# Luckick/EAGCN

Hardware: AMD Instinct MI355X
Metric: molecules/sec fwd+bwd, 2-layer 5-view EAGCN, Tox21 batch (higher is better)
Workload: dtype f32 (bf16x3 split, fp32 accumulate): every fp32 operand leaves its producer as three bf16 planes, six v_mfma_f32_32x32x16_bf16 piece products per 16 k rebuild the fp32 product (csrc/gemm_bx3.hip); aggregation, BatchNorm, head, first layer fp32

## Files before the change

eagcn_amd/_lib.py:

```python
import ctypes as C
import os

_HERE = os.path.dirname(os.path.abspath(__file__))
LIB_PATH = os.path.join(_HERE, 'lib', 'libeagcn_hip.so')

MAX_VIEWS = 8
MAX_SEGS = 8
META_WORDS = 16
META_NLOG = 8
META_T, META_NMAX, META_NTILES, META_BAD_ADJ, META_BAD_REL, META_NEDGE, META_OVERFLOW, META_EDGE_OVERFLOW = range(8)
META_NBLK = 9
STRUCT_CONCATE, STRUCT_WEIGHTED = 0, 1

_fp = C.c_void_p


class Batch(C.Structure):
    _fields_ = [('B', C.c_int32), ('N', C.c_int32), ('K', C.c_int32), ('ldc', C.c_int32),
                ('T', C.c_int32), ('n_max', C.c_int32), ('n_tiles', C.c_int32),
                ('channels', C.c_int32 * MAX_VIEWS),
                ('code', _fp), ('deg_bn', _fp), ('nat', _fp), ('row0', _fp), ('tile0', _fp),
                ('meta', _fp), ('row_mol', _fp), ('row_loc', _fp), ('row_m', _fp), ('row_deg', _fp),
                ('tile_mol', _fp), ('row_info', _fp), ('tile_info', _fp),
                ('rel_vec', _fp * MAX_VIEWS), ('rel_c', C.c_int32 * MAX_VIEWS),
# ... 176 lines not shown
    'eagcn_stream_signal_flag': (C.c_int, [_fp, _fp]),
    'eagcn_stream_wait_flag': (C.c_int, [_fp, C.c_double, _fp]),
    'eagcn_stream_wait_timeouts': (C.c_int, []),
    'eagcn_stream_wait_reset': (None, []),
    'eagcn_adam_step': (C.c_int, [_fp, _fp, _fp, _fp, C.c_int64, _fp, _fp, _fp, _fp]),
    'eagcn_grad_norm_workspace_bytes': (C.c_size_t, []),
    'eagcn_grad_norm': (C.c_int, [_fp, _fp, C.c_int64, _fp, C.c_int, _fp]),
    'eagcn_adam_step_clipped': (C.c_int, [_fp, _fp, _fp, _fp, C.c_int64, _fp, _fp, _fp, _fp, _fp, _fp, _fp]),
    'eagcn_agg_wants_bond_lists': (C.c_int, [C.c_int, C.c_int]),
    'eagcn_agg_wants_bond_lists_for': (C.c_int, [C.c_int, C.c_int, C.c_int]),
    'eagcn_bx3_used_splits': (C.c_int, [C.c_int, C.c_int, C.c_int, C.c_int]),
    'eagcn_set_bx3_wide': (C.c_int, [C.c_int]),
    'eagcn_set_top_bn_sums': (C.c_int, [C.c_int]),
    'eagcn_set_hidden_bn_sums': (C.c_int, [C.c_int]),
    'eagcn_hidden_bn_sums_taken': (C.c_long, [C.c_int]),
    'eagcn_bx3_pair_used_splits': (C.c_int, [C.c_int] * 7),
    'eagcn_bx3_plane_elems': (C.c_size_t, [C.c_int, C.c_int]),
    'eagcn_bx3_split': (C.c_int, [_fp, C.c_int, C.c_int, _fp, C.c_size_t, C.c_int, C.c_int, _fp]),
    'eagcn_gemm_bx3': (C.c_int, [C.c_int, C.c_int, C.c_int, C.c_int, _fp, C.c_size_t, C.c_int, C.c_int, _fp, C.c_size_t, C.c_int, C.c_int,
                                 _fp, C.c_int, C.c_int, C.c_size_t, C.c_int, _fp]),
    'eagcn_gemm_bx3_pair': (C.c_int, [C.c_int, C.c_int, C.c_int, _fp, C.c_size_t, C.c_int, C.c_int, _fp, C.c_size_t, C.c_int, C.c_int, _fp, C.c_int,
                                      C.c_int, C.c_int, C.c_int, _fp, C.c_size_t, C.c_int, C.c_int, _fp, C.c_size_t, C.c_int, C.c_int, _fp, C.c_int,
                                      C.c_int, C.c_size_t, C.c_int, _fp]),
    'eagcn_pack_rows': (C.c_int, [C.POINTER(Batch), _fp, C.c_int, C.POINTER(Layout), _fp, _fp]),
    'eagcn_unpack_rows': (C.c_int, [C.POINTER(Batch), _fp, C.POINTER(Layout), _fp, _fp, C.c_int, _fp]),
    'eagcn_pad_rows': (C.c_int, [_fp, _fp, C.c_int, C.c_int, C.c_int, _fp, _fp]),
    'eagcn_gat_scratch_bytes': (C.c_size_t, [C.POINTER(Batch), C.c_int]),
    'eagcn_gat_forward': (C.c_int, [C.POINTER(Batch), C.POINTER(GatParams), _fp, _fp, _fp, _fp, _fp]),
    'eagcn_gat_backward': (C.c_int, [C.POINTER(Batch), C.POINTER(GatParams), _fp, _fp, _fp, _fp, _fp, _fp, _fp, _fp, _fp,
                                     C.c_size_t, _fp]),
# ... 145 lines not shown
```

eagcn_amd/build.py:

```python
import os
import shutil
import subprocess
import sys
from concurrent.futures import ThreadPoolExecutor

HERE = os.path.dirname(os.path.abspath(__file__))
CSRC = os.path.join(HERE, 'csrc')
LIBDIR = os.path.join(HERE, 'lib')
LIB = os.path.join(LIBDIR, 'libeagcn_hip.so')
HIP_SOURCES = ['index.hip', 'gemm.hip', 'gemm3.hip', 'gemm_bx3.hip', 'gemm_bx3w.hip', 'agg.hip', 'lagg.hip', 'lagg_in.hip', 'lagg_top.hip', 'gat.hip', 'pool.hip', 'layer.hip', 'readout.hip', 'head.hip', 'head2.hip', 'loss.hip', 'clip.hip', 'attr.hip', 'metrics.hip', 'reps.hip']
CPP_SOURCES = ['api.cpp']
HEADERS = ['common.h', 'kernels.h', 'lagg_kernel.h', 'gemm_x6.h', 'bx3.h', 'bx3_epi.h', os.path.join('..', '..', 'include', 'eagcn_hip.h')]
ARCH = 'gfx950'


def _hipcc():
    for cand in (shutil.which('hipcc'), '/opt/rocm/bin/hipcc'):
        if cand and os.path.exists(cand):
            return cand
    raise RuntimeError('hipcc not found: the EAGCN HIP library cannot be built')


def _newest(paths):
    return max(os.path.getmtime(p) for p in paths)

# ... 46 lines not shown
```

eagcn_amd/csrc/kernels.h:

```cpp
#pragma once
#include "bx3.h"
#include "common.h"

namespace eagcn {

struct AggArgs {
    eagcn_batch bt;
    ViewCols vc;
    const float* src; int lds;
    float* dst; int ldd;
    const float* sig;
    const float* rsig;
    float* rscale;
    double* stats;
    int nchunk;
    int cpw = 1;
    int xcd = 0;
    bool w_rowm = false;
    bool w_gather = false;
    BxOut planes = {nullptr, 0, 0, 0};
    const float* bn_tab = nullptr; const float* bn_cc = nullptr; int bn_fp = 0;
    const float* w_aw = nullptr;
    int w_drop = 0; uint32_t w_thr = 0; float w_inv_keep = 1.0f; uint64_t w_seed = 0; const uint64_t* w_seed_dev = nullptr;
};
struct DropArgs { int on; uint32_t thr; float inv_keep; uint64_t seed; const uint64_t* seed_dev; };
inline DropArgs drop_args(float p, bool training, uint64_t seed, const uint64_t* seed_dev) {
    const double thr = (double)p * 4294967296.0;
    return DropArgs{(training && p > 0.0f) ? 1 : 0, (uint32_t)(thr < 4294967295.0 ? thr : 4294967295.0), 1.0f / (1.0f - p), seed, seed_dev};
}
inline void agg_set_drop(AggArgs& a, const DropArgs& d) {
    a.w_drop = d.on; a.w_thr = d.thr; a.w_inv_keep = d.inv_keep; a.w_seed = d.seed; a.w_seed_dev = d.seed_dev;
}
int agg_grid_x(const eagcn_batch* b);
bool agg_ksplit(const eagcn_batch* b);
int launch_agg(AggArgs a, bool trans, hipStream_t s);
constexpr int LAGG_RB = 256;
constexpr int LAGG_MAXM = 16;
struct EdgeArgs;
int lagg_parts();
bool lagg_wfuse();
bool lagg_use(const eagcn_batch* b, int dir, bool absorbs_bn, const ViewCols* vc = nullptr);
bool lagg_wanted(int B, int N, int structure);
int lagg_block_rows(const eagcn_batch* b);
int lagg_slabs(const eagcn_batch* b);
int launch_lagg_fwd(AggArgs a, hipStream_t s);
int launch_lagg_bwd(AggArgs a, const EdgeArgs& e, hipStream_t s, bool edge = true);
int launch_lagg_bwd_input(const AggArgs& a, const EdgeArgs& e, dim3 grid, hipStream_t s);
int launch_lagg_bwd_top(const AggArgs& a, const EdgeArgs& e, dim3 grid, hipStream_t s);

struct EdgeArgs {
    eagcn_batch bt;
    ViewCols vc;
    const float* dY; const float* Y; const float* P; int ld;
    const float* sig; const float* rsig; const float* rscale;
    double* datt;
    int atomic;
    int xcd = 0;
};
constexpr int EDGE_SLAB = 264;
constexpr int EDGE_COPIES = 8;
inline size_t edge_acc_bytes() { return align256((size_t)EDGE_COPIES * EAGCN_MAX_VIEWS * EDGE_SLAB * sizeof(double)); }
int edge_grid_x(const eagcn_batch* b);
int launch_agg_edge(AggArgs a, const EdgeArgs& e, hipStream_t s);
// ... 213 lines not shown
```

eagcn_amd/csrc/lagg.hip:

```cpp
#include <stdlib.h>

#include <algorithm>

#include "common.h"
#include "kernels.h"
#include "lagg_kernel.h"

namespace eagcn {


static int lagg_cpw(const eagcn_batch& bt, const ViewCols& vc, bool trans);
static int lagg_policy() {
    static const int v = [] {
        const char* e = getenv("EAGCN_AGG");
        if (e && !strcmp(e, "lds")) return 1;
        if (e && !strcmp(e, "dense")) return 0;
        return 2;
    }();
    return v;
}
static int lagg_min_n() {
    static const int v = env_int("EAGCN_LAGG_MIN_N", 240);
    return v;
}
// ... 46 lines not shown
    int chunks, gy;
    lagg_extent(bt, vc, &chunks, &gy);
    const long wgs = (long)vc.K * chunks * gy;
    int per = (trans && !cpw_bwd) ? 1 : cpw_env > 0 ? cpw_env : (int)std::min<long>(trans ? 4 : 8, std::max<long>(1, wgs / 3072));
    return std::max(1, std::min(per, chunks));
}
static int lagg_grid(const AggArgs& a, dim3* grid, int* nchunk, int* cpw, bool trans) {
    int chunks, gy;
    lagg_extent(a.bt, a.vc, &chunks, &gy);
    *cpw = lagg_cpw(a.bt, a.vc, trans);
    *nchunk = cdiv(chunks, *cpw);
    *grid = dim3((unsigned)(a.vc.K * *nchunk), (unsigned)gy);
    return EAGCN_OK;
}

int launch_lagg_fwd(AggArgs a, hipStream_t s) {
    if (a.bt.B == 0 || a.bt.T == 0) return EAGCN_OK;
    dim3 grid;
    int rc = lagg_grid(a, &grid, &a.nchunk, &a.cpw, false);
    if (rc) return rc;
    ProfScope ps(PROF_AGG, s);
    EdgeArgs e;
    memset(&e, 0, sizeof(e));
    if (a.cpw > 1) lagg_kernel<false, true><<<grid, 256, 0, s>>>(a, e);
    else lagg_kernel<false, false><<<grid, 256, 0, s>>>(a, e);
    EAGCN_LAUNCH_CHECK();
    return EAGCN_OK;
}

int launch_lagg_bwd(AggArgs a, const EdgeArgs& e, hipStream_t s, bool edge) {
    if (a.bt.B == 0 || a.bt.T == 0) return EAGCN_OK;
    EAGCN_CHECK_ARG(!edge || (e.atomic && e.datt), "lagg: the edge gradients leave through the shared accumulator slabs (EdgeArgs.atomic)");
    dim3 grid;
    int rc = lagg_grid(a, &grid, &a.nchunk, &a.cpw, true);
    if (rc) return rc;
    ProfScope ps(PROF_AGG, s);
    EAGCN_CHECK_ARG(!a.w_aw || a.bn_tab, "lagg: the upstream-gradient form needs the BatchNorm tables");
    EAGCN_CHECK_ARG(!a.w_rowm || a.bn_tab, "lagg: the row-mask staging needs the BatchNorm tables");
    if (!edge) {
        rc = launch_lagg_bwd_input(a, e, grid, s);
        if (rc) return rc;
    } else if (a.w_rowm) {
        rc = launch_lagg_bwd_top(a, e, grid, s);
        if (rc) return rc;
    } else if (a.w_aw) {
        lagg_kernel<true, true, true><<<grid, 256, 0, s>>>(a, e);
    } else {
        if (a.cpw > 1) lagg_kernel<true, true><<<grid, 256, 0, s>>>(a, e);
        else lagg_kernel<true, false><<<grid, 256, 0, s>>>(a, e);
    }
    EAGCN_LAUNCH_CHECK();
    return EAGCN_OK;
}

}

extern "C" int eagcn_agg_wants_bond_lists(int B, int N) { return eagcn::lagg_wanted(B, N, -1) ? 1 : 0; }
extern "C" int eagcn_agg_wants_bond_lists_for(int B, int N, int structure) { return eagcn::lagg_wanted(B, N, structure) ? 1 : 0; }
```

eagcn_amd/csrc/lagg_kernel.h:

```cpp
#pragma once

#include "common.h"
#include "kernels.h"

namespace eagcn {

constexpr int LG_CW = 32;
constexpr int LG_LPR = LG_CW / 4;
constexpr int LG_G = 256 / LG_LPR;
constexpr int LG_U = LAGG_RB / LG_G;
constexpr int LG_ECAP = 768;
constexpr int LG_EPT = LG_ECAP / 256;
constexpr bool LG_MERGE = true;
constexpr int LG_PJ_EARLY = 4;

__device__ __forceinline__ void lg_fma(float4& acc, float w, const float4& v) {
    acc.x = fmaf(w, v.x, acc.x); acc.y = fmaf(w, v.y, acc.y); acc.z = fmaf(w, v.z, acc.z); acc.w = fmaf(w, v.w, acc.w);
}
__device__ __forceinline__ void lg_add(float4& acc, const float4& v) { acc.x += v.x; acc.y += v.y; acc.z += v.z; acc.w += v.w; }
__device__ __forceinline__ float lg_dot(const float4& a, const float4& b) { return fmaf(a.x, b.x, fmaf(a.y, b.y, fmaf(a.z, b.z, a.w * b.w))); }
template <int CTRL>
__device__ __forceinline__ float lg_dpp(float v) {
    return __int_as_float(__builtin_amdgcn_update_dpp(0, __float_as_int(v), CTRL, 0xF, 0xF, true));
}
__device__ __forceinline__ float lg_gsum(float v) {
    v += lg_dpp<0xB1>(v); v += lg_dpp<0x4E>(v); v += lg_dpp<0x141>(v);
    return v;
}

struct LgLists {
    unsigned short nb[LG_ECAP];
    float w[LG_ECAP];
    unsigned char cd[LG_ECAP];
};
constexpr uint32_t LG_SLOW = 1u << 28;
constexpr uint32_t LG_OVF = 1u << 29;
constexpr int LG_NOVF = 32;

template <bool TRANS, bool MULTI, bool WFUSE = false, bool EDGE = true, bool CROWS = false, bool GATHER = false>
__global__ __launch_bounds__(256) __attribute__((amdgpu_waves_per_eu(3, 8))) void lagg_kernel(AggArgs a, EdgeArgs ed) {
    static_assert(TRANS || !WFUSE, "the upstream-gradient form belongs to the transposed kernel");
    static_assert(TRANS || EDGE, "the forward has no edge gradients to drop");
    static_assert(!CROWS || WFUSE, "the row-mask staging is a form of the upstream-gradient staging");
    static_assert(!GATHER || (CROWS && EDGE && MULTI), "the per-molecule gather is a form of the row-mask staging with the edge gradients");
    constexpr bool TE = TRANS && EDGE;
    constexpr int NREC = TRANS ? 3 : 2;
    __shared__ float4 buf[LAGG_RB][LG_LPR];
    __shared__ float4 s_rec[LAGG_RB][NREC];
    __shared__ float4 s_ovf[LG_NOVF][NREC];
    __shared__ int s_novf;
    __shared__ __attribute__((aligned(16))) unsigned char s_lists_raw[TRANS ? 16 : sizeof(LgLists)];
    __shared__ float s_rs[TRANS ? LAGG_RB : 1];
    __shared__ float s_rd[TE ? LAGG_RB : 1];
    __shared__ unsigned char s_rm[LAGG_RB];
    __shared__ float4 s_S[LAGG_MAXM][LG_LPR];
// ... 43 lines not shown
        const int cl = cc * LG_CW + tid < wk ? a.vc.off[k] + cc * LG_CW + tid : a.vc.off[k];
        const float sc = a.bn_tab[(size_t)BN_SC * a.bn_fp + cl], mu = a.bn_tab[(size_t)BN_MU * a.bn_fp + cl];
        const bool no_cc = !EDGE && a.bn_cc == nullptr;
        const float iv = a.bn_tab[(size_t)BN_INV * a.bn_fp + cl], c1 = no_cc ? 0.0f : a.bn_cc[cl], c2 = no_cc ? 0.0f : a.bn_cc[a.bn_fp + cl];
        float* sb = reinterpret_cast<float*>(&s_bn[0][0]);
        sb[tid] = sc;
        sb[LG_CW + tid] = -sc * iv * c2;
        sb[2 * LG_CW + tid] = sc * (mu * iv * c2 - c1);
        if constexpr (WFUSE) sb[3 * LG_CW + tid] = a.bn_tab[(size_t)BN_SH * a.bn_fp + cl];
    };
    const float w_ave = (WFUSE && !CROWS) ? a.w_aw[a.vc.off[k]] : 0.0f;
    const uint64_t wseed = WFUSE && a.w_drop ? (a.w_seed_dev ? *a.w_seed_dev : a.w_seed) : 0ull;
    if constexpr (TRANS) {
        if (fuse_bn && tid < LG_CW) bn_consts(cc_lo);
    }
    for (int q = blockIdx.y; q < nblk; q += gridDim.y) {
        const int4 b0 = b0n, b1 = b1n;
        asm volatile("" : "+v"(g));
        if (q + (int)gridDim.y < nblk) { b0n = blk4[2 * (q + gridDim.y)]; b1n = blk4[2 * (q + gridDim.y) + 1]; }
        const int m0 = b0.x, R0 = b0.z, rows = min(b0.w, LAGG_RB), E0 = b1.x, ne = b1.y;
        if (rows <= 0) {
            if constexpr (!TRANS) {
                const int fp = a.vc.off[a.vc.K];
                for (int cc = cc_lo; cc < cc_hi; ++cc)
                    if (tid < LG_CW && cc * LG_CW + tid < wk)
                        *reinterpret_cast<double2*>(a.stats + ((size_t)q * fp + a.vc.off[k] + cc * LG_CW + tid) * 2) = make_double2(0.0, 0.0);
            }
            continue;
        }
        const int nst = min(ne, LG_ECAP);
// ... 325 lines not shown
            if constexpr (!TRANS) {
                s1[0] += (double)y.x; s2[0] += (double)y.x * (double)y.x;
                s1[1] += (double)y.y; s2[1] += (double)y.y * (double)y.y;
                s1[2] += (double)y.z; s2[2] += (double)y.z * (double)y.z;
                s1[3] += (double)y.w; s2[3] += (double)y.w * (double)y.w;
                if (col_ok) *reinterpret_cast<float4*>(a.dst + (size_t)(R0 + rr) * a.ldd + c0) = y;
            } else {
                if (col_ok) {
                    int cs = c0;
                    asm volatile("" : "+v"(cs));
                    if (a.planes.p) bx_store4(a.planes, R0 + rr, cs, y);
                    else *reinterpret_cast<float4*>(a.dst + (size_t)(R0 + rr) * a.ldd + cs) = y;
                }
            }
        };
        bool any_slow = false;
        {
            constexpr bool AHEAD = !TRANS;
            float4 nrec[NREC];
            if constexpr (AHEAD) {
#pragma unroll
                for (int i = 0; i < NREC; ++i) nrec[i] = s_rec[min(g, rows - 1)][i];
            }
            const int nu = (rows + LG_G - 1) / LG_G;
#pragma unroll
            for (int u = 0; u < LG_U; ++u) {
                if (u >= nu) break;
                const int rr = min(g + LG_G * u, rows - 1);
                const bool valid = g + LG_G * u < rows;
                if constexpr (!AHEAD) {
#pragma unroll
                    for (int i = 0; i < NREC; ++i) nrec[i] = s_rec[rr][i];
                }
                const float4 r0 = nrec[0], r1 = nrec[1], rl = nrec[NREC - 1];
                if (AHEAD && u + 1 < LG_U) {
#pragma unroll
                    for (int i = 0; i < NREC; ++i) nrec[i] = s_rec[min(rr + LG_G, rows - 1)][i];
                }
                const uint32_t srcs = __float_as_uint(TRANS ? rl.y : rl.z), meta = __float_as_uint(rl.w);
                const bool fast = valid && !(meta & LG_SLOW);
                any_slow = any_slow || (valid && (meta & LG_SLOW));
                const float4 self = buf[rr][l];
// ... 24 lines not shown
                    const uint32_t sr2 = __float_as_uint(TRANS ? s_ovf[slot][NREC - 1].y : s_ovf[slot][NREC - 1].z);
                    const float4 b0 = buf[sr2 & 255u][l], b1 = buf[(sr2 >> 8) & 255u][l], b2 = buf[(sr2 >> 16) & 255u][l], b3 = buf[sr2 >> 24][l];
                    lg_fma(y, q0.x, b0); lg_fma(y, q0.y, b1); lg_fma(y, q0.z, b2); lg_fma(y, q0.w, b3);
                    if constexpr (TE && LG_MERGE) {
                        const float4 pj = col_ok ? pjv[u] : make_float4(0.f, 0.f, 0.f, 0.f);
                        const float4 q1 = s_ovf[slot][1];
                        const uint32_t cd2 = __float_as_uint(s_ovf[slot][2].z);
                        const float f0 = lg_gsum(lg_dot(b0, pj)), f1 = lg_gsum(lg_dot(b1, pj)), f2 = lg_gsum(lg_dot(b2, pj)), f3 = lg_gsum(lg_dot(b3, pj));
                        const int e4 = l & 3;
                        const float hv2 = e4 == 0 ? q1.x : e4 == 1 ? q1.y : e4 == 2 ? q1.z : q1.w;
                        const float gv2 = e4 == 0 ? f0 : e4 == 1 ? f1 : e4 == 2 ? f2 : f3;
                        const uint32_t cv2 = (cd2 >> (8 * e4)) & 255u, sv2 = (sr2 >> (8 * e4)) & 255u;
                        if (l < 4 && hv2 != 0.0f && cv2) atomicAdd(&h_s[cv2], (double)hv2 * ((double)gv2 - (double)s_rd[sv2]));
                    }
                }
                if (fast) finish(rr, y);
            }
        }
        if (any_slow) {
#pragma unroll 1
            for (int u = 0; u < LG_U; ++u) {
                const int rr = g + LG_G * u;
                if (rr >= rows) break;
                const float4 r1 = s_rec[rr][1], rl = s_rec[rr][NREC - 1];
                const uint32_t srcs = __float_as_uint(TRANS ? rl.y : rl.z), meta = __float_as_uint(rl.w);
                if (!(meta & LG_SLOW)) continue;
                const int cnt_r = (int)((meta >> 16) & 255u), first_r = (int)(meta & 0xFFFFu);
                const float4 self = buf[rr][l];
                const float4 S = s_S[(meta >> 24) & 15u][l];
                int jn0; float w0; uint32_t cq;
                entry(first_r, !TRANS, jn0, w0, cq);
// ... 31 lines not shown
                                if (c) atomicAdd(&h_s[c], (double)(dU * w * (1.0f - w)));
                                if (src == rr) dr_acc += (double)dU;
                            }
                        }
                        self_bond = self_bond || src == rr;
                    }
                    y.x = acc.x + rs * self.x + TINY * (S.x - bs.x);
                    y.y = acc.y + rs * self.y + TINY * (S.y - bs.y);
                    y.z = acc.z + rs * self.z + TINY * (S.z - bs.z);
                    y.w = acc.w + rs * self.w + TINY * (S.w - bs.w);
                    if constexpr (EDGE) {
                        const float gs = lg_gsum(lg_dot(self, pj));
                        if (l == 0 && sj != 0.0f && !self_bond) dr_acc += (double)(sj * (gs - s_rd[rr]));
                    }
                }
                finish(rr, y);
            }
        }
        if constexpr (!TRANS) {
#pragma unroll
            for (int e = 0; e < 4; ++e) {
#pragma unroll
                for (int o = LG_LPR; o < 64; o <<= 1) { s1[e] += __shfl_xor(s1[e], o); s2[e] += __shfl_xor(s2[e], o); }
            }
            if (lane < LG_LPR) {
#pragma unroll
                for (int e = 0; e < 4; ++e) { st_s[wave][lane][2 * e] = s1[e]; st_s[wave][lane][2 * e + 1] = s2[e]; }
            }
            __syncthreads();
            if (tid < LG_CW && cc * LG_CW + tid < wk) {
                const int fp = a.vc.off[a.vc.K];
                const int ll = tid >> 2, e = tid & 3;
                const double t1 = (st_s[0][ll][2 * e] + st_s[1][ll][2 * e]) + (st_s[2][ll][2 * e] + st_s[3][ll][2 * e]);
                const double t2 = (st_s[0][ll][2 * e + 1] + st_s[1][ll][2 * e + 1]) + (st_s[2][ll][2 * e + 1] + st_s[3][ll][2 * e + 1]);
                *reinterpret_cast<double2*>(a.stats + ((size_t)q * fp + a.vc.off[k] + cc * LG_CW + tid) * 2) = make_double2(t1, t2);
            }
        }
        }
    }
    if constexpr (TE) {
        if (dr_acc != 0.0) atomicAdd(&h_s[256], dr_acc);
        __syncthreads();
        double* out = ed.datt + ((size_t)((blockIdx.y + blockIdx.x) & (EDGE_COPIES - 1)) * ed.vc.K + k) * EDGE_SLAB;
        int te = tid;
        if constexpr (GATHER) asm volatile("" : "+v"(te));
        const double hv = h_s[te];
        if (hv != 0.0) atomicAdd(&out[te], hv);
        if (tid == 0 && h_s[256] != 0.0) atomicAdd(&out[256], h_s[256]);
    }
}

}
// ... 1 lines not shown
```

eagcn_amd/csrc/layer.hip:

```cpp
#include <algorithm>

#include <stdlib.h>

#include "common.h"
#include "kernels.h"

namespace eagcn {

struct ParamPtrs {
    const float* att_w[EAGCN_MAX_VIEWS];
    const float* self_r[EAGCN_MAX_VIEWS];
    const float* W[EAGCN_MAX_VIEWS];
    const float* bias[EAGCN_MAX_VIEWS];
    const float* gamma[EAGCN_MAX_VIEWS];
    const float* beta[EAGCN_MAX_VIEWS];
    float* run_mean[EAGCN_MAX_VIEWS];
    float* run_var[EAGCN_MAX_VIEWS];
    const float* ave_w;
    int channels[EAGCN_MAX_VIEWS];
    const float* rel_vec[EAGCN_MAX_VIEWS];
    int rel_c[EAGCN_MAX_VIEWS];
};
__device__ __forceinline__ float att_logit(const ParamPtrs& pp, int k, int c) {
    if (!pp.rel_vec[k]) return pp.att_w[k][c - 1];
// ... 539 lines not shown
        const float4 iv = *reinterpret_cast<const float4*>(bn + BN_INV * fp + c);
        const float4 c1 = *reinterpret_cast<const float4*>(cc + c);
        const float4 c2 = *reinterpret_cast<const float4*>(cc + fp + c);
        d.x = sc.x * (d.x - c1.x - (y.x - mu.x) * iv.x * c2.x);
        d.y = sc.y * (d.y - c1.y - (y.y - mu.y) * iv.y * c2.y);
        d.z = sc.z * (d.z - c1.z - (y.z - mu.z) * iv.z * c2.z);
        d.w = sc.w * (d.w - c1.w - (y.w - mu.w) * iv.w * c2.w);
        *reinterpret_cast<float4*>(dH + (size_t)r * fp + c) = d;
    }
}

__global__ __launch_bounds__(256) void unpack_grads_kernel(GradPtrs gp, ParamPtrs pp, ViewCols vc, ColMapD in,
                                                            int ld_in, int fp, const float* __restrict__ dWcat,
                                                            int nsplit, size_t slab, double* __restrict__ datt,
                                                            int nedge, const float* __restrict__ rsig, int wblocks,
                                                            const int32_t* __restrict__ meta, int xk_G, int edge_drain, int bx_per, int bx_wide) {
    nedge = nedge < 0 ? -nedge : min(nedge, (meta[EAGCN_META_T] + 15) / 16);
    const int bxm = bx_wide ? BX3W_BM : BX3_BM, bxn = bx_wide ? BX3W_BN : BX3_BN;
    nsplit = nsplit < 0 ? bx3_used_splits_wave(-nsplit, meta[EAGCN_META_T], ((ld_in + bxm - 1) / bxm) * ((fp + bxn - 1) / bxn),
                                          bx_per > 0 ? ((meta[EAGCN_META_T] + bxm - 1) / bxm) * ((ld_in + bxn - 1) / bxn) : 0, max(1, (fp + 31) >> 5), bx_per)
                        : max(1, min(nsplit, meta[EAGCN_META_T] >> 7));
    if ((int)blockIdx.x < wblocks) {
        const int tid = blockIdx.x * blockDim.x + threadIdx.x;
        if (xk_G > 0) {
            const int e = tid;
            if (e >= ld_in * fp) return;
            const int ip = e / fp, cp = e % fp;
            const int k = col_view(vc, cp), f = cp - vc.off[k];
            const int fi = packed_to_exact(in, ip);
            if (fi < 0 || f >= vc.width[k]) return;
            const int T = meta[EAGCN_META_T];
            G3Plan pl;
            g3_plan((T + 63) / 64, (ld_in + 63) / 64, max(1, (fp + 15) / 16), ((ld_in + 63) / 64) * ((fp + 63) / 64),
                    max(1, (T + 15) / 16), xk_G, pl);
            float v[G3_XSEG];
// ... 305 lines not shown
    bool has_drain_out;
    bool top_sums = false;
    bool top_gather = false;
    bool dh_given = false;
};
struct LayerRoute {
    FwdProd fwd_prod = FWD_NONE; bool fwd_split_x = false;
    AggPath fwd_agg = AGG_DENSE, bwd_agg = AGG_DENSE;
    Bn2 bn2 = BN2_NONE;
    bool rows_first = false, rows_late = false;
    bool store_dh = false;
    EdgePath edge = EDGE_NONE; bool edge_atomic = false;
    BwdProd bwd_prod = BWD_NONE; bool bwd_split_x = false;
    bool defer_drain = false;
    bool dh_given = false;
    bool bn2_staged() const { return bn2 >= BN2_STAGED_FROM_DH; }
    bool bwd_planes() const { return bwd_prod >= BWD_PLANES_PAIR && bwd_prod <= BWD_PLANES_DX; }
};

static bool sw_gemm3() { static const bool on = !env_flag("EAGCN_NO_GEMM3", false); return on; }
static bool sw_planes_only() { static const bool on = env_flag("EAGCN_PLANES_ONLY", true); return on; }
static bool bn_bwd_two_pass(bool weighted) {
    static const int force = getenv("EAGCN_BWD_STORE_DH") ? (env_flag("EAGCN_BWD_STORE_DH", false) ? 1 : 0) : -1;
    return force < 0 ? weighted : force == 0;
}
static bool gemm3_layer(int ld_in) {
    return sw_gemm3() && ld_in >= 128 && gemm_mode() != 2;
}

static LayerRoute plan_layer(const eagcn_batch* b, const eagcn_layer_params* p, const eagcn_layer_bufs* w, const LayerDims& d,
                             PlanAsk ask) {
    LayerRoute r;
    const bool wt = p->structure == EAGCN_STRUCT_WEIGHTED;
    bool general = false;
    for (int k = 0; k < p->K; ++k) general = general || b->rel_vec[k] != nullptr;
    r.edge_atomic = !general;
    r.store_dh = !bn_bwd_two_pass(wt);
    if (b->T <= 0) return r;
    r.fwd_agg = fwd_agg_lagg(b, d.vc) ? AGG_LAGG : AGG_DENSE;
    float* const some_dx = reinterpret_cast<float*>(static_cast<uintptr_t>(4096));
    LayerScratch sc;
    carve_layer(w->scratch, b, d, true, &sc);
    if (w->packed) carve_packed(w->packed, d, &sc.pk);
// ... 24 lines not shown
        r.store_dh = false;
    }

    r.dh_given = ask.dh_given && r.bn2 == BN2_STAGED_FROM_DH && r.store_dh && !wt && !ask.mol_grad && !ask.input_only;
    const bool planes = d.np && bx3_ok(bq.bw) && (!ask.has_dx || bx3_ok(bq.bx));
    r.bwd_split_x = planes && !w->x_planes && !ask.input_only;
    if (ask.input_only) r.bwd_prod = planes ? BWD_PLANES_DX : BWD_TILED_DX;
    else if (!planes && !w->x) r.bwd_prod = BWD_REFUSED;
    if (r.bwd_prod != BWD_NONE) return r;
    r.edge = (lagg && r.edge_atomic) ? EDGE_WITH_LAGG : EDGE_COLAUNCH;
    if (planes) r.bwd_prod = ask.has_dx ? BWD_PLANES_PAIR : BWD_PLANES_DW;
    else if (ask.has_dx && gemm3_layer(d.ld_in) && gemm3_ok(gq.gw) && gemm3_ok(gq.gx))
        r.bwd_prod = gemm3_xk_enabled() ? BWD_G3_XK : BWD_G3_SCATTER;
    else r.bwd_prod = ask.has_dx ? BWD_TILED_PAIR : BWD_TILED_SEPARATE;
    r.defer_drain = ask.has_drain_out && r.edge_atomic && r.bwd_prod == BWD_G3_SCATTER;
    return r;
}

static int apply_launch(const eagcn_batch* b, const eagcn_layer_params* p, const eagcn_layer_bufs* w, const LayerDims& d,
                        const float* colp, hipStream_t s, bool planes_only = false) {
    ProfScope psbn(PROF_BN, s);
    ApplyArgs aa;
    aa.bt = *b; aa.vc = d.vc; aa.structure = p->structure; aa.fp = d.fp; aa.Y = w->Y; aa.ldy = d.fp;
    aa.bn = w->bn; aa.colp = colp; aa.out = w->xout; aa.ldo = d.ldo; aa.pad_row = w->pad_row;
    const DropArgs dr = drop_args(p->dropout, p->training != 0, p->seed, p->seed_dev);
    aa.do_drop = dr.on; aa.thr = dr.thr; aa.inv_keep = dr.inv_keep; aa.seed = dr.seed; aa.seed_dev = dr.seed_dev;
    aa.planes = BxOut{gemm_planes() ? w->xout_planes : nullptr, bx_plane_elems(b->T, d.ldo), gemm_planes(), b->T};
    if (planes_only && aa.planes.p) aa.out = nullptr;
    aa.tile_map = aa.planes.p ? 1 : 0;
    const size_t nthr = aa.tile_map ? (size_t)cdiv(std::max(b->T, 1), 8) * cdiv(d.ldo, 32) * 64 : (size_t)std::max(b->T, 1) * d.ldo / 4;
// ... 174 lines not shown
extern "C" int eagcn_set_top_bn_sums(int on) {
    const int old = g_top_bn_sums;
    g_top_bn_sums = on == 2 ? 2 : on ? 1 : 0;
    return old;
}
static int g_hidden_bn_sums = env_flag("EAGCN_HIDDEN_BN_SUMS", true) ? 1 : 0;
static long g_hidden_bn_taken = 0;
extern "C" long eagcn_hidden_bn_sums_taken(int reset) {
    const long n = g_hidden_bn_taken;
    if (reset) g_hidden_bn_taken = 0;
    return n;
}
extern "C" int eagcn_set_hidden_bn_sums(int on) {
    const int old = g_hidden_bn_sums;
    g_hidden_bn_sums = on ? 1 : 0;
    return old;
}
bool eagcn::layer_hidden_sums_route(const eagcn_batch* b, const eagcn_layer_params* up, const eagcn_layer_params* low, BxBnEpi* ep) {
    if (!g_hidden_bn_sums || !b || !up || !low || b->T <= 0 || low->structure != EAGCN_STRUCT_CONCATE || !low->training) return false;
    void* const some = reinterpret_cast<void*>(static_cast<uintptr_t>(4096));
    eagcn_layer_bufs w;
    memset(&w, 0, sizeof(w));
    w.x_planes = static_cast<const uint16_t*>(some); w.x = static_cast<const float*>(some); w.P = static_cast<float*>(some); w.scratch = some;
    const LayerDims du = layer_dims(b, up), dl = layer_dims(b, low);
    if (du.ld_in != dl.fp || dl.ldo != dl.fp || hidden_bn_slabs(b->T) > dl.gxb) return false;
    const LayerRoute ru = plan_layer(b, up, &w, du, PlanAsk{true, false, false, false});
    const LayerRoute rl = plan_layer(b, low, &w, dl, PlanAsk{true, false, false, false, false, false, true});
    if (ru.bwd_prod != BWD_PLANES_PAIR || !rl.dh_given || rl.bwd_agg != AGG_LAGG) return false;
    if (ep) {
        memset(ep, 0, sizeof(*ep));
// ... 148 lines not shown
    EAGCN_LAUNCH_CHECK();
    return EAGCN_OK;
}

static int bwd_aggregate(LayerBwd& c) {
    const eagcn_batch* b = c.b; const eagcn_layer_bufs* w = c.w; const LayerDims& d = c.d; const LayerScratch& sc = c.sc;
    const LayerRoute& r = c.r; hipStream_t s = c.s;
    AggArgs a;
    a.bt = *b; a.vc = d.vc; a.src = sc.dY; a.lds = d.fp; a.dst = sc.dP; a.ldd = d.fp;
    a.sig = sc.pk.sig; a.rsig = sc.pk.rsig; a.rscale = w->rscale; a.stats = nullptr; a.nchunk = 1;
    if (r.bwd_planes()) a.planes = BxOut{sc.dPp, bx_plane_elems(b->T, d.fp), d.np, b->T};
    if (r.bn2_staged()) {
        a.bn_tab = w->bn; a.bn_cc = (c.o.input_only && !c.p->training) ? nullptr : sc.cc; a.bn_fp = d.fp;
    }
    if (r.dh_given) { a.src = c.dxout; a.lds = d.ldo; }
    if (r.bn2 == BN2_STAGED_FROM_UPSTREAM || r.bn2 == BN2_STAGED_ROWMASK || r.bn2 == BN2_STAGED_FROM_READOUT) {
        a.src = c.dg ? sc.dY : c.dxout; a.lds = d.ldo;
        a.w_aw = sc.pk.colp + (size_t)CP_AVEW * d.fp;
        a.w_rowm = r.bn2 != BN2_STAGED_FROM_UPSTREAM;
        if (r.bn2 == BN2_STAGED_FROM_READOUT && !r.rows_late) { a.src = c.o.top_dge; a.lds = c.o.rg->F; a.w_gather = true; }
        agg_set_drop(a, c.drop);
    }
    EdgeArgs e;
    e.bt = *b; e.vc = d.vc; e.dY = sc.dY; e.Y = w->Y; e.P = w->P; e.ld = d.fp; e.sig = sc.pk.sig;
    e.rsig = sc.pk.rsig; e.rscale = w->rscale; e.datt = r.edge_atomic ? sc.eacc : sc.datt; e.atomic = r.edge_atomic ? 1 : 0;
    switch (r.edge) {
    case EDGE_NONE:
        return r.bwd_agg == AGG_LAGG ? launch_lagg_bwd(a, e, s, false) : launch_agg(a, true, s);
    case EDGE_WITH_LAGG: return launch_lagg_bwd(a, e, s);
    default: return launch_agg_edge(a, e, s);
    }
}

static int bwd_products(LayerBwd& c, const LayerOperands& o) {
    const eagcn_batch* b = c.b; const LayerDims& d = c.d; const LayerScratch& sc = c.sc; hipStream_t s = c.s;
    const PlaneProducts bq = layer_plane_products(b, d, o);
    const Fp32Products gq = layer_fp32_products(b, d, o, c.gemm_work);
    DwScatter dsc;
    for (int k = 0; k < EAGCN_MAX_VIEWS; ++k) dsc.dW[k] = c.gp.dW[k];
    dsc.vc = d.vc;
    dsc.in = c.in;
    int rc;
    c.nsplit = d.nsplit;
    switch (c.r.bwd_prod) {
    case BWD_PLANES_DX: return launch_bx3(bq.bx, nullptr, d.np, s, c.gemm_work, PROF_GEMM, bx3_pick_wide(bq.bx, nullptr, b->t_hint));
    case BWD_TILED_DX: return launch_gemm(gq.gx, s);
    case BWD_PLANES_PAIR: {
        c.bx_wide = bx3_pick_wide(bq.bx, &bq.bw, b->t_hint);
        BxProb bx = bq.bx;
        if (c.o.below && !c.bx_wide) {
            EAGCN_CHECK_ARG(c.o.below->Y && c.o.below->bn && c.o.below->row_m && c.o.below->slab && c.o.below->fp == bx.N && bx.ldc == bx.N,
                            "eagcn_layer_backward: incomplete description of the layer below");
            EAGCN_CHECK_ARG((bx.N & 3) == 0 && (c.o.below->ldy & 3) == 0 && (reinterpret_cast<uintptr_t>(c.o.below->slab) & 15) == 0,
                            "eagcn_layer_backward: the tail pass of the dX product needs packed widths that are multiples of 4");
            bx.ep = *c.o.below;
            if (c.o.below_done) *c.o.below_done = true;
        }
        rc = launch_bx3(bx, &bq.bw, d.np, s, 2.0 * c.gemm_work, PROF_GEMM_PAIR, c.bx_wide);
// ... 28 lines not shown
        for (int k = 0; k < p->K; ++k)
            { int rcz = zero_fill(c.gp.dW[k], (size_t)d.fin * p->width[k] * sizeof(float), c.s); if (rcz) return rcz; }
    }
    if (c.r.defer_drain) {
        EdgeDrain* out = c.o.drain_out;
        out->eacc = sc.eacc; out->K = p->K; out->rsig = sc.pk.rsig;
        for (int k = 0; k < EAGCN_MAX_VIEWS; ++k) {
            out->datt_w[k] = c.gp.datt_w[k]; out->dself_r[k] = c.gp.dself_r[k]; out->channels[k] = c.pp.channels[k];
        }
        return EAGCN_OK;
    }
    const int wblocks = c.nsplit > 0 ? cdiv((int)d.wslab, 256) : 0;
    const bool shared = b->T > 0 && c.r.edge_atomic;
    const int nedge = b->T > 0 ? (shared ? -EDGE_COPIES : edge_grid_x(b)) : 0;
    ProfScope psu(PROF_PACK, c.s);
    unpack_grads_kernel<<<wblocks + cdiv(p->K * EDGE_SLAB, 16), 256, 0, c.s>>>(c.gp, c.pp, d.vc, c.in, d.ld_in, d.fp, sc.dWcat,
                                                                                  c.bx_slabs ? -c.nsplit : c.nsplit, d.wslab,
                                                                                  shared ? sc.eacc : sc.datt, nedge, sc.pk.rsig,
                                                                                  wblocks, b->meta, c.xk_G, shared ? 1 : 0, c.bx_per, c.bx_wide);
    EAGCN_LAUNCH_CHECK();
    return EAGCN_OK;
}

int eagcn::layer_backward_impl(const eagcn_batch* b, const eagcn_layer_params* p, const eagcn_layer_bufs* w,
                               const float* dxout, const float* dpad_row, float* dx, const eagcn_layer_grads* g, void* stream,
                               const LayerBwdOpts& o) {
    if (o.drain_out) o.drain_out->eacc = nullptr;
    int rc = check_layer(b, p, "eagcn_layer_backward");
    if (rc) return rc;
    EAGCN_CHECK_ARG(w && (g || o.input_only) && w->bn && w->scratch, "eagcn_layer_backward: null buffer");
    EAGCN_CHECK_ARG(!o.input_only || (dx && !o.drain_in), "eagcn_layer_backward: the input-only form needs dx and takes no edge reduction");
    EAGCN_CHECK_ARG(b->T == 0 || ((dxout || o.rg) && (o.input_only || w->x || w->x_planes) && w->P && w->Y && w->rscale),
                    "eagcn_layer_backward: null activation buffer");
    if (!o.input_only)
// ... 78 lines not shown
```

include/eagcn_hip.h:

```cpp
#ifndef EAGCN_HIP_H
#define EAGCN_HIP_H

#include <stddef.h>
#include <stdint.h>

#ifdef __cplusplus
extern "C" {
#endif

#define EAGCN_MAX_VIEWS 8
#define EAGCN_MAX_SEGS 8
#define EAGCN_MAX_CHANNELS 255
#define EAGCN_STRUCT_CONCATE 0
#define EAGCN_STRUCT_WEIGHTED 1

#define EAGCN_OK 0
#define EAGCN_ERR_ARG (-1)
#define EAGCN_ERR_HIP (-2)
#define EAGCN_ERR_SCRATCH (-3)

#define EAGCN_META_T 0
#define EAGCN_META_NMAX 1
#define EAGCN_META_NTILES 2
#define EAGCN_META_BAD_ADJ 3
// ... 317 lines not shown
                       size_t workspace_bytes, void* stream);
int eagcn_kmeans_iterate(const float* X, int64_t n, int F, int ld, int k, void* workspace, size_t workspace_bytes, void* stream);
int eagcn_kmeans_finish(const float* X, int64_t n, int F, int ld, int k, void* workspace, size_t workspace_bytes, void* stream);
int eagcn_kmeans_assign(const float* X, int64_t n, int F, int ld, const float* centers, int k, int32_t* labels, float* mind,
                        void* workspace, size_t workspace_bytes, void* stream);

int eagcn_set_gemm_mode(int mode);

size_t eagcn_bx3_plane_elems(int rows_cap, int ld);
int eagcn_bx3_split(const float* x, int rows, int ld, uint16_t* planes, size_t plane_stride, int rows_cap, int np, void* stream);
int eagcn_bx3_used_splits(int splits, int M, int N, int K);
int eagcn_set_bx3_wide(int mode);
int eagcn_set_top_bn_sums(int on);
int eagcn_set_hidden_bn_sums(int on);
long eagcn_hidden_bn_sums_taken(int reset);
int eagcn_bx3_pair_used_splits(int splits, int M, int N, int K, int M0, int N0, int K0);
int eagcn_gemm_bx3(int tn, int M, int N, int K, const uint16_t* A, size_t a_pstride, int lda, int a_rows, const uint16_t* B,
                   size_t b_pstride, int ldb, int b_rows, float* C, int ldc, int splits, size_t slab, int np, void* stream);
int eagcn_gemm_bx3_pair(int M0, int N0, int K0, const uint16_t* A0, size_t a0_pstride, int lda0, int a0_rows, const uint16_t* B0,
                        size_t b0_pstride, int ldb0, int b0_rows, float* C0, int ldc0, int M1, int N1, int K1, const uint16_t* A1,
                        size_t a1_pstride, int lda1, int a1_rows, const uint16_t* B1, size_t b1_pstride, int ldb1, int b1_rows,
                        float* C1, int ldc1, int splits, size_t slab, int np, void* stream);

int eagcn_gemm_f32(int ta, int tb, int M, int N, int K, const float* A, int lda, const float* B,
                   int ldb, float* C, int ldc, void* stream);
int eagcn_gemm_f32_dev(int ta, int tb, int M, int N, int K, const float* A, int lda, const float* B,
                       int ldb, float* C, int ldc, const int32_t* extent_dev, int which, void* stream);

size_t eagcn_gemm_sk_workspace_bytes(void);
int eagcn_gemm_f32_sk(int ta, int tb, int M, int N, int K, const float* A, int lda, const float* B, int ldb, float* C,
// ... 24 lines not shown
```

Measured before the change: 749,900.

## Fuse first-layer weight-gradient GEMM into the transposed aggregation backward kernel

```diff
diff --git a/eagcn_amd/_lib.py b/eagcn_amd/_lib.py
--- a/eagcn_amd/_lib.py
+++ b/eagcn_amd/_lib.py
@@ -214,6 +214,9 @@
     'eagcn_set_top_bn_sums': (C.c_int, [C.c_int]),
     'eagcn_set_hidden_bn_sums': (C.c_int, [C.c_int]),
     'eagcn_hidden_bn_sums_taken': (C.c_long, [C.c_int]),
+    'eagcn_set_first_layer_fused': (C.c_int, [C.c_int]),
+    'eagcn_first_layer_fused_taken': (C.c_long, [C.c_int]),
+    'eagcn_first_layer_fused_last': (None, [C.POINTER(C.c_int32)]),
     'eagcn_bx3_pair_used_splits': (C.c_int, [C.c_int] * 7),
     'eagcn_bx3_plane_elems': (C.c_size_t, [C.c_int, C.c_int]),
     'eagcn_bx3_split': (C.c_int, [_fp, C.c_int, C.c_int, _fp, C.c_size_t, C.c_int, C.c_int, _fp]),
diff --git a/eagcn_amd/build.py b/eagcn_amd/build.py
--- a/eagcn_amd/build.py
+++ b/eagcn_amd/build.py
@@ -8,7 +8,7 @@
 CSRC = os.path.join(HERE, 'csrc')
 LIBDIR = os.path.join(HERE, 'lib')
 LIB = os.path.join(LIBDIR, 'libeagcn_hip.so')
-HIP_SOURCES = ['index.hip', 'gemm.hip', 'gemm3.hip', 'gemm_bx3.hip', 'gemm_bx3w.hip', 'agg.hip', 'lagg.hip', 'lagg_in.hip', 'lagg_top.hip', 'gat.hip', 'pool.hip', 'layer.hip', 'readout.hip', 'head.hip', 'head2.hip', 'loss.hip', 'clip.hip', 'attr.hip', 'metrics.hip', 'reps.hip']
+HIP_SOURCES = ['index.hip', 'gemm.hip', 'gemm3.hip', 'gemm_bx3.hip', 'gemm_bx3w.hip', 'agg.hip', 'lagg.hip', 'lagg_in.hip', 'lagg_top.hip', 'lagg_dw.hip', 'gat.hip', 'pool.hip', 'layer.hip', 'readout.hip', 'head.hip', 'head2.hip', 'loss.hip', 'clip.hip', 'attr.hip', 'metrics.hip', 'reps.hip']
 CPP_SOURCES = ['api.cpp']
 HEADERS = ['common.h', 'kernels.h', 'lagg_kernel.h', 'gemm_x6.h', 'bx3.h', 'bx3_epi.h', os.path.join('..', '..', 'include', 'eagcn_hip.h')]
 ARCH = 'gfx950'
diff --git a/eagcn_amd/csrc/kernels.h b/eagcn_amd/csrc/kernels.h
--- a/eagcn_amd/csrc/kernels.h
+++ b/eagcn_amd/csrc/kernels.h
@@ -22,6 +22,7 @@
     const float* bn_tab = nullptr; const float* bn_cc = nullptr; int bn_fp = 0;
     const float* w_aw = nullptr;
     int w_drop = 0; uint32_t w_thr = 0; float w_inv_keep = 1.0f; uint64_t w_seed = 0; const uint64_t* w_seed_dev = nullptr;
+    const float* fx = nullptr; int fx_ld = 0; float* dw = nullptr; size_t dw_slab = 0; int dw_ny = 0;
 };
 struct DropArgs { int on; uint32_t thr; float inv_keep; uint64_t seed; const uint64_t* seed_dev; };
 inline DropArgs drop_args(float p, bool training, uint64_t seed, const uint64_t* seed_dev) {
@@ -47,6 +48,8 @@
 int launch_lagg_bwd(AggArgs a, const EdgeArgs& e, hipStream_t s, bool edge = true);
 int launch_lagg_bwd_input(const AggArgs& a, const EdgeArgs& e, dim3 grid, hipStream_t s);
 int launch_lagg_bwd_top(const AggArgs& a, const EdgeArgs& e, dim3 grid, hipStream_t s);
+int launch_lagg_bwd_dw(const AggArgs& a, const EdgeArgs& e, dim3 grid, hipStream_t s);
+int lagg_bwd_grid_y(const eagcn_batch* b, const ViewCols& vc);
 
 struct EdgeArgs {
     eagcn_batch bt;
diff --git a/eagcn_amd/csrc/lagg.hip b/eagcn_amd/csrc/lagg.hip
--- a/eagcn_amd/csrc/lagg.hip
+++ b/eagcn_amd/csrc/lagg.hip
@@ -84,6 +84,12 @@
     return EAGCN_OK;
 }
 
+int lagg_bwd_grid_y(const eagcn_batch* b, const ViewCols& vc) {
+    int chunks, gy;
+    lagg_extent(*b, vc, &chunks, &gy);
+    return gy;
+}
+
 int launch_lagg_fwd(AggArgs a, hipStream_t s) {
     if (a.bt.B == 0 || a.bt.T == 0) return EAGCN_OK;
     dim3 grid;
@@ -113,6 +119,10 @@
     } else if (a.w_rowm) {
         rc = launch_lagg_bwd_top(a, e, grid, s);
         if (rc) return rc;
+    } else if (a.dw) {
+        grid.y = (unsigned)std::max(1, std::min((int)grid.y, a.dw_ny));
+        rc = launch_lagg_bwd_dw(a, e, grid, s);
+        if (rc) return rc;
     } else if (a.w_aw) {
         lagg_kernel<true, true, true><<<grid, 256, 0, s>>>(a, e);
     } else {
diff --git a/eagcn_amd/csrc/lagg_dw.hip b/eagcn_amd/csrc/lagg_dw.hip
--- /dev/null
+++ b/eagcn_amd/csrc/lagg_dw.hip
@@ -0,0 +1,14 @@
+#include "lagg_kernel.h"
+
+namespace eagcn {
+
+int launch_lagg_bwd_dw(const AggArgs& a, const EdgeArgs& e, dim3 grid, hipStream_t s) {
+    EAGCN_CHECK_ARG(a.fx && a.dw && a.fx_ld >= 1 && a.fx_ld <= LG_CW && a.dw_ny >= 1 && (int)grid.y == a.dw_ny && !a.planes.p && !a.w_aw,
+                    "lagg: the weight-gradient epilogue takes at most 32 input columns and one slab per workgroup row");
+    if (a.cpw > 1) lagg_kernel<true, true, false, true, false, false, true><<<grid, 256, 0, s>>>(a, e);
+    else lagg_kernel<true, false, false, true, false, false, true><<<grid, 256, 0, s>>>(a, e);
+    EAGCN_LAUNCH_CHECK();
+    return EAGCN_OK;
+}
+
+}
diff --git a/eagcn_amd/csrc/lagg_kernel.h b/eagcn_amd/csrc/lagg_kernel.h
--- a/eagcn_amd/csrc/lagg_kernel.h
+++ b/eagcn_amd/csrc/lagg_kernel.h
@@ -37,8 +37,9 @@
 constexpr uint32_t LG_OVF = 1u << 29;
 constexpr int LG_NOVF = 32;
 
-template <bool TRANS, bool MULTI, bool WFUSE = false, bool EDGE = true, bool CROWS = false, bool GATHER = false>
+template <bool TRANS, bool MULTI, bool WFUSE = false, bool EDGE = true, bool CROWS = false, bool GATHER = false, bool DWF = false>
 __global__ __launch_bounds__(256) __attribute__((amdgpu_waves_per_eu(3, 8))) void lagg_kernel(AggArgs a, EdgeArgs ed) {
+    static_assert(!DWF || (TRANS && EDGE && !WFUSE), "the weight-gradient epilogue belongs to the plain transposed kernel with the edge gradients");
     static_assert(TRANS || !WFUSE, "the upstream-gradient form belongs to the transposed kernel");
     static_assert(TRANS || EDGE, "the forward has no edge gradients to drop");
     static_assert(!CROWS || WFUSE, "the row-mask staging is a form of the upstream-gradient staging");
@@ -112,6 +113,14 @@
     if constexpr (TRANS) {
         if (fuse_bn && tid < LG_CW) bn_consts(cc_lo);
     }
+    int nacc = 0;
+    auto dw_out = [&](int cc, int i, float t, bool first) __attribute__((always_inline)) {
+        const int e = tid + 256 * i, m = e >> 5, cv = cc * LG_CW + (e & 31);
+        if (m < a.fx_ld && cv < wk) {
+            float* dp = a.dw + (size_t)blockIdx.y * a.dw_slab + (size_t)m * a.vc.off[a.vc.K] + a.vc.off[k] + cv;
+            *dp = first ? t : *dp + t;
+        }
+    };
     for (int q = blockIdx.y; q < nblk; q += gridDim.y) {
         const int4 b0 = b0n, b1 = b1n;
         asm volatile("" : "+v"(g));
@@ -467,6 +476,7 @@
                 }
             }
         };
+        float4 ys[DWF ? LG_U : 1];
         bool any_slow = false;
         {
             constexpr bool AHEAD = !TRANS;
@@ -478,7 +488,7 @@
             const int nu = (rows + LG_G - 1) / LG_G;
 #pragma unroll
             for (int u = 0; u < LG_U; ++u) {
-                if (u >= nu) break;
+                if (!DWF && u >= nu) break;
                 const int rr = min(g + LG_G * u, rows - 1);
                 const bool valid = g + LG_G * u < rows;
                 if constexpr (!AHEAD) {
@@ -533,7 +543,8 @@
                         if (l < 4 && hv2 != 0.0f && cv2) atomicAdd(&h_s[cv2], (double)hv2 * ((double)gv2 - (double)s_rd[sv2]));
                     }
                 }
-                if (fast) finish(rr, y);
+                if constexpr (DWF) ys[u] = fast ? y : make_float4(0.f, 0.f, 0.f, 0.f);
+                else { if (fast) finish(rr, y); }
             }
         }
         if (any_slow) {
@@ -595,7 +606,59 @@
                         if (l == 0 && sj != 0.0f && !self_bond) dr_acc += (double)(sj * (gs - s_rd[rr]));
                     }
                 }
-                finish(rr, y);
+                if constexpr (DWF) {
+#pragma unroll
+                    for (int q8 = 0; q8 < LG_U; ++q8)
+                        if (q8 == u) ys[q8] = y;
+                } else finish(rr, y);
+            }
+        }
+        if constexpr (DWF) {
+            float* bf = reinterpret_cast<float*>(&buf[0][0]);
+            const int li = lane & 15, kq = lane >> 4;
+            __syncthreads();
+#pragma unroll
+            for (int u = 0; u < LG_U; ++u) buf[g + LG_G * u][l] = ys[u];
+            float xa[16][2];
+            int rq = 64 * wave + kq;
+            asm volatile("" : "+v"(rq));
+            {
+                const uint32_t c0x = (uint32_t)min(li, a.fx_ld - 1), c1x = (uint32_t)min(16 + li, a.fx_ld - 1);
+#pragma unroll
+                for (int ks = 0; ks < 16; ++ks) {
+                    const uint32_t ro = (uint32_t)(R0 + min(rq + 4 * ks, rows - 1)) * (uint32_t)a.fx_ld;
+                    xa[ks][0] = a.fx[ro + c0x];
+                    xa[ks][1] = a.fx[ro + c1x];
+                }
+            }
+            __syncthreads();
+            typedef float lg_f32x4 __attribute__((ext_vector_type(4)));
+            lg_f32x4 acc[2][2];
+#pragma unroll
+            for (int i = 0; i < 2; ++i)
+#pragma unroll
+                for (int j = 0; j < 2; ++j) acc[i][j] = lg_f32x4{0.f, 0.f, 0.f, 0.f};
+#pragma unroll
+            for (int ks = 0; ks < 16; ++ks) {
+                const float b0 = bf[(rq + 4 * ks) * LG_CW + li], b1 = bf[(rq + 4 * ks) * LG_CW + 16 + li];
+                acc[0][0] = __builtin_amdgcn_mfma_f32_16x16x4f32(xa[ks][0], b0, acc[0][0], 0, 0, 0);
+                acc[0][1] = __builtin_amdgcn_mfma_f32_16x16x4f32(xa[ks][0], b1, acc[0][1], 0, 0, 0);
+                acc[1][0] = __builtin_amdgcn_mfma_f32_16x16x4f32(xa[ks][1], b0, acc[1][0], 0, 0, 0);
+                acc[1][1] = __builtin_amdgcn_mfma_f32_16x16x4f32(xa[ks][1], b1, acc[1][1], 0, 0, 0);
+            }
+            __syncthreads();
+#pragma unroll
+            for (int i = 0; i < 2; ++i)
+#pragma unroll
+                for (int j = 0; j < 2; ++j)
+#pragma unroll
+                    for (int rr4 = 0; rr4 < 4; ++rr4)
+                        bf[wave * 1024 + (16 * i + 4 * kq + rr4) * LG_CW + 16 * j + li] = acc[i][j][rr4];
+            __syncthreads();
+#pragma unroll
+            for (int i = 0; i < 4; ++i) {
+                const int e = tid + 256 * i;
+                dw_out(cc, i, (bf[e] + bf[1024 + e]) + (bf[2048 + e] + bf[3072 + e]), nacc == 0);
             }
         }
         if constexpr (!TRANS) {
@@ -617,6 +680,14 @@
                 *reinterpret_cast<double2*>(a.stats + ((size_t)q * fp + a.vc.off[k] + cc * LG_CW + tid) * 2) = make_double2(t1, t2);
             }
         }
+        }
+        if constexpr (DWF) ++nacc;
+    }
+    if constexpr (DWF) {
+        if (nacc == 0) {
+            for (int cc = cc_lo; cc < cc_hi; ++cc)
+#pragma unroll
+                for (int i = 0; i < 4; ++i) dw_out(cc, i, 0.0f, true);
         }
     }
     if constexpr (TE) {
diff --git a/eagcn_amd/csrc/layer.hip b/eagcn_amd/csrc/layer.hip
--- a/eagcn_amd/csrc/layer.hip
+++ b/eagcn_amd/csrc/layer.hip
@@ -577,11 +577,13 @@
                                                             int ld_in, int fp, const float* __restrict__ dWcat,
                                                             int nsplit, size_t slab, double* __restrict__ datt,
                                                             int nedge, const float* __restrict__ rsig, int wblocks,
-                                                            const int32_t* __restrict__ meta, int xk_G, int edge_drain, int bx_per, int bx_wide) {
+                                                            const int32_t* __restrict__ meta, int xk_G, int edge_drain, int bx_per, int bx_wide,
+                                                            int all_slabs) {
     nedge = nedge < 0 ? -nedge : min(nedge, (meta[EAGCN_META_T] + 15) / 16);
     const int bxm = bx_wide ? BX3W_BM : BX3_BM, bxn = bx_wide ? BX3W_BN : BX3_BN;
     nsplit = nsplit < 0 ? bx3_used_splits_wave(-nsplit, meta[EAGCN_META_T], ((ld_in + bxm - 1) / bxm) * ((fp + bxn - 1) / bxn),
                                           bx_per > 0 ? ((meta[EAGCN_META_T] + bxm - 1) / bxm) * ((ld_in + bxn - 1) / bxn) : 0, max(1, (fp + 31) >> 5), bx_per)
+                        : all_slabs ? nsplit
                         : max(1, min(nsplit, meta[EAGCN_META_T] >> 7));
     if ((int)blockIdx.x < wblocks) {
         const int tid = blockIdx.x * blockDim.x + threadIdx.x;
@@ -917,6 +919,7 @@
     BwdProd bwd_prod = BWD_NONE; bool bwd_split_x = false;
     bool defer_drain = false;
     bool dh_given = false;
+    bool dw_fused = false; int dw_ny = 0; bool dw_in_dp = false;
     bool bn2_staged() const { return bn2 >= BN2_STAGED_FROM_DH; }
     bool bwd_planes() const { return bwd_prod >= BWD_PLANES_PAIR && bwd_prod <= BWD_PLANES_DX; }
 };
@@ -930,6 +933,10 @@
 static bool gemm3_layer(int ld_in) {
     return sw_gemm3() && ld_in >= 128 && gemm_mode() != 2;
 }
+static int g_first_layer_fused = env_flag("EAGCN_FIRST_LAYER_FUSED", true) ? 1 : 0;
+static long g_first_layer_fused_taken = 0;
+static int32_t g_first_layer_fused_last[3] = {0, 0, 0};
+static bool first_layer_fused_enabled() { return g_first_layer_fused != 0; }
 
 static LayerRoute plan_layer(const eagcn_batch* b, const eagcn_layer_params* p, const eagcn_layer_bufs* w, const LayerDims& d,
                              PlanAsk ask) {
@@ -984,6 +991,15 @@
         r.bwd_prod = gemm3_xk_enabled() ? BWD_G3_XK : BWD_G3_SCATTER;
     else r.bwd_prod = ask.has_dx ? BWD_TILED_PAIR : BWD_TILED_SEPARATE;
     r.defer_drain = ask.has_drain_out && r.edge_atomic && r.bwd_prod == BWD_G3_SCATTER;
+    const bool plain_staging = r.bn2 != BN2_STAGED_FROM_UPSTREAM && r.bn2 != BN2_STAGED_ROWMASK && r.bn2 != BN2_STAGED_FROM_READOUT;
+    if (first_layer_fused_enabled() && r.bwd_prod == BWD_TILED_SEPARATE && r.edge == EDGE_WITH_LAGG && r.bwd_agg == AGG_LAGG &&
+        plain_staging && d.ld_in <= 32 && gemm_mode() != 1 && gemm_mode() != 2 && w->x) {
+        const long cap_w = std::max(std::max(d.nsplit, G3_XSEG), d.np ? d.bx_splits : 1);
+        const long cap_p = (long)(((size_t)std::max(b->T, 1) * d.fp) / d.wslab);
+        r.dw_fused = true;
+        r.dw_ny = (int)std::max<long>(1, std::min<long>(lagg_bwd_grid_y(b, d.vc), std::max(cap_w, cap_p)));
+        r.dw_in_dp = r.dw_ny > cap_w;
+    }
     return r;
 }
 
@@ -1188,6 +1204,17 @@
 extern "C" int eagcn_set_hidden_bn_sums(int on) {
     const int old = g_hidden_bn_sums;
     g_hidden_bn_sums = on ? 1 : 0;
+    return old;
+}
+extern "C" long eagcn_first_layer_fused_taken(int reset) {
+    const long n = g_first_layer_fused_taken;
+    if (reset) g_first_layer_fused_taken = 0;
+    return n;
+}
+extern "C" void eagcn_first_layer_fused_last(int32_t out[3]) { memcpy(out, g_first_layer_fused_last, sizeof(g_first_layer_fused_last)); }
+extern "C" int eagcn_set_first_layer_fused(int on) {
+    const int old = g_first_layer_fused;
+    g_first_layer_fused = on ? 1 : 0;
     return old;
 }
 bool eagcn::layer_hidden_sums_route(const eagcn_batch* b, const eagcn_layer_params* up, const eagcn_layer_params* low, BxBnEpi* ep) {
@@ -1366,6 +1393,11 @@
         a.bn_tab = w->bn; a.bn_cc = (c.o.input_only && !c.p->training) ? nullptr : sc.cc; a.bn_fp = d.fp;
     }
     if (r.dh_given) { a.src = c.dxout; a.lds = d.ldo; }
+    if (r.dw_fused) {
+        ++g_first_layer_fused_taken;
+        g_first_layer_fused_last[0] = r.dw_ny; g_first_layer_fused_last[1] = r.dw_in_dp ? 1 : 0; g_first_layer_fused_last[2] = lagg_bwd_grid_y(b, d.vc);
+        a.dst = nullptr; a.fx = w->x; a.fx_ld = d.ld_in; a.dw = r.dw_in_dp ? sc.dP : sc.dWcat; a.dw_slab = d.wslab; a.dw_ny = r.dw_ny;
+    }
     if (r.bn2 == BN2_STAGED_FROM_UPSTREAM || r.bn2 == BN2_STAGED_ROWMASK || r.bn2 == BN2_STAGED_FROM_READOUT) {
         a.src = c.dg ? sc.dY : c.dxout; a.lds = d.ldo;
         a.w_aw = sc.pk.colp + (size_t)CP_AVEW * d.fp;
@@ -1394,6 +1426,10 @@
     dsc.in = c.in;
     int rc;
     c.nsplit = d.nsplit;
+    if (c.r.dw_fused) {
+        c.nsplit = c.r.dw_ny;
+        return EAGCN_OK;
+    }
     switch (c.r.bwd_prod) {
     case BWD_PLANES_DX: return launch_bx3(bq.bx, nullptr, d.np, s, c.gemm_work, PROF_GEMM, bx3_pick_wide(bq.bx, nullptr, b->t_hint));
     case BWD_TILED_DX: return launch_gemm(gq.gx, s);
@@ -1452,10 +1488,12 @@
     const bool shared = b->T > 0 && c.r.edge_atomic;
     const int nedge = b->T > 0 ? (shared ? -EDGE_COPIES : edge_grid_x(b)) : 0;
     ProfScope psu(PROF_PACK, c.s);
-    unpack_grads_kernel<<<wblocks + cdiv(p->K * EDGE_SLAB, 16), 256, 0, c.s>>>(c.gp, c.pp, d.vc, c.in, d.ld_in, d.fp, sc.dWcat,
+    unpack_grads_kernel<<<wblocks + cdiv(p->K * EDGE_SLAB, 16), 256, 0, c.s>>>(c.gp, c.pp, d.vc, c.in, d.ld_in, d.fp,
+                                                                                  (c.r.dw_fused && c.r.dw_in_dp) ? sc.dP : sc.dWcat,
                                                                                   c.bx_slabs ? -c.nsplit : c.nsplit, d.wslab,
                                                                                   shared ? sc.eacc : sc.datt, nedge, sc.pk.rsig,
-                                                                                  wblocks, b->meta, c.xk_G, shared ? 1 : 0, c.bx_per, c.bx_wide);
+                                                                                  wblocks, b->meta, c.xk_G, shared ? 1 : 0, c.bx_per, c.bx_wide,
+                                                                                  c.r.dw_fused ? 1 : 0);
     EAGCN_LAUNCH_CHECK();
     return EAGCN_OK;
 }
diff --git a/include/eagcn_hip.h b/include/eagcn_hip.h
--- a/include/eagcn_hip.h
+++ b/include/eagcn_hip.h
@@ -355,6 +355,9 @@
 int eagcn_set_top_bn_sums(int on);
 int eagcn_set_hidden_bn_sums(int on);
 long eagcn_hidden_bn_sums_taken(int reset);
+int eagcn_set_first_layer_fused(int on);
+long eagcn_first_layer_fused_taken(int reset);
+void eagcn_first_layer_fused_last(int32_t out[3]);
 int eagcn_bx3_pair_used_splits(int splits, int M, int N, int K, int M0, int N0, int K0);
 int eagcn_gemm_bx3(int tn, int M, int N, int K, const uint16_t* A, size_t a_pstride, int lda, int a_rows, const uint16_t* B,
                    size_t b_pstride, int ldb, int b_rows, float* C, int ldc, int splits, size_t slab, int np, void* stream);
```

Result: faster. 772,100 (median of 6 runs) (+3.0%).
